# shrubb/latent-pose-reenactment

Measured on AMD Instinct MI355X. Metric: train-step images/sec at 256x256 bs=8, higher is better.
Workload: dtype mixed 16-bit MFMA operands, fp32 accumulate, fp32 activations / weights / optimizer state; 1 GPU; default.yaml meta-training step (configs[2]): ResNeXt50 identity encoder over 8 frames + MobileNetV2 pose encoder (both trained, forward + backward on hand-written gfx950 kernels), G, D with the 98000x512 label embedding, VGG19/VGGFace/featmat/adversarial/dis_embed/dice criterions, Adam, EMA; image_size=256, per_gpu_batch=8, global_batch=8, parallelism=dp1, precision_mode=default assignment (LP_PREC=f16), padding=zero, launch_mode=hipgraph

## Files before the change

include/lp_hip.h:

```cpp
#ifndef LP_HIP_H
#define LP_HIP_H
#include <stdint.h>
#ifdef __cplusplus
extern "C" {
#endif

#define LP_OK 0
#define LP_ERR_ARG (-1)
#define LP_ERR_UNSUPPORTED (-2)
#define LP_ERR_HIP (-3)

#define LP_PREC_BF16 0
#define LP_PREC_BF16X3 1
#define LP_PREC_F16 2

const char* lp_last_error(void);
int lp_abi_version(void);

int lp_pack_weights(const float* w, uint16_t* hi, uint16_t* lo, int Cout, int Cin, int T, int RowsP, int ColsP, int mode, int f16,
                    void* stream);
int lp_pack_desc_bytes(void);
int lp_pack_weights_batch(const void* table, int num_entries, long long total_chunks, void* stream);
int lp_pack_pair_desc_bytes(void);
int lp_pack_weights_pairs(const void* table, int num_entries, long long total_tiles, void* stream);
// ... 184 lines not shown
int lp_reduce_dice(const float* fake, const float* real, float* partial, float* out, float* sums, int B, int Cf, int Cr, int HW,
                   float weight, void* stream);
int lp_reduce_dice_bwd(const float* fake, const float* real, const float* sums, const float* grad_out, float* dfake, int B, int Cf,
                       int Cr, int HW, float weight, void* stream);
int lp_reduce_hinge(const float* real, const float* fake_d, const float* fake_g, float* out, int B, void* stream);
int lp_reduce_hinge_bwd(const float* real, const float* fake_d, const float* grad_G, const float* grad_D, float* d_real,
                        float* d_fake_d, float* d_fake_g, int B, void* stream);

int lp_proj_score_fwd(const float* out, const float* embed, float* pooled, float* dot, int N, int HW, int C, void* stream);
int lp_proj_score_bwd(const float* out, const float* embed, const float* pooled, const float* g_pooled, const float* g_dot, float* d_out,
                      float* d_embed, int N, int HW, int C, void* stream);
int lp_embed_tail_fwd(const float* out, float* elem, float* embeds, int* argk, int B, int K, int HW, int C, int is_max, void* stream);
int lp_embed_tail_bwd(const float* out, const float* g_elem, const float* g_embeds, const int* argk, float* d_out, int B, int K, int HW, int C,
                      int is_max, void* stream);
int lp_stem8_supported(int Cin, int Cout, int ksize, int W);
int lp_stem8_fwd(const float* xa, const long long* stride_a, int Ca, const float* xb, const long long* stride_b, int Cb, int cmap,
                 const uint16_t* w_hi, const uint16_t* w_lo, float* y, const float* bias, const float* alpha, int N, int H, int W, int Cin,
                 int Cout, int CinP, int CoutP, int ksize, int prec, uint16_t* out_hi, uint16_t* out_lo, int out_relu, void* stream);
long long lp_stem8_wgrad_workspace_bytes(int N, int H, int Cout, int ksize);
int lp_stem8_wgrad(const float* xa, const long long* stride_a, int Ca, const float* xb, const long long* stride_b, int Cb, int cmap,
                   const float* dy, float* dw, float* dbias, float* workspace, int N, int H, int W, int Cin, int Cout, int ksize, void* stream);
int lp_stem8_dgrad(const float* dy, const float* w, const float* alpha, float* dx, const long long* stride_dx, int Cb, int cmap, int N, int H,
                   int W, int Cin, int Cout, int ksize, void* stream);
int lp_image_prep_fwd(const float* x, const float* mean, const float* stdv, float* out, int N, int HW, void* stream);
int lp_image_prep_bwd(const float* g, const float* stdv, float* dx, int N, int HW, void* stream);
int lp_stickman_render(const float* points, int N, int P, const int* seg, const int* part_end, const float* colour, int L, int parts, int S,
                       float width, float* out, void* stream);

int lp_mt_desc_bytes(void);
int lp_mt_optimizer_step(const void* table, int num_tensors, long long max_numel, long long* step, int kind, float lr,
                         float beta1, float beta2, float eps, void* stream);
int lp_mt_ema(const void* table, int num_tensors, long long max_numel, float alpha, int copy_only, void* stream);

int lp_sn_desc_bytes(void);
int lp_sn_row_block(void);
int lp_sn_power_iter(const void* table, int num_layers, int do_iter, int max_rows, int max_cols, void* stream);
int lp_sn_grad_apply(float* g, const float* w_orig, const float* u, const float* v, const float* sig, float* dot, int ndot,
                     float* accum, int rows, int cols, void* stream);
int lp_sn_apply_desc_bytes(void);
int lp_sn_grad_apply_batch(const void* host_descs, int count, void* stream);
int lp_sn_embed_grad(float* grad, const float* u, const float* v, const float* coef, const long long* label, const float* rows,
                     int N, int E, int B, void* stream);

#ifdef __cplusplus
}
#endif
// ... 2 lines not shown
```

latent_pose_reenactment_amd/_lib.py:

```python
import ctypes
import os

import torch

_HERE = os.path.dirname(os.path.abspath(__file__))
LIB_PATH = os.environ.get('LP_LIB_OVERRIDE') or os.path.join(_HERE, 'liblp_hip.so')

PREC_BF16 = 0
PREC_BF16X3 = 1
PREC_F16 = 2

_vp, _i, _f, _ll = ctypes.c_void_p, ctypes.c_int, ctypes.c_float, ctypes.c_longlong

SIGNATURES = {
    'lp_last_error': (ctypes.c_char_p, []),
    'lp_abi_version': (_i, []),
    'lp_pack_weights': (_i, [_vp, _vp, _vp, _i, _i, _i, _i, _i, _i, _i, _vp]),
    'lp_pack_desc_bytes': (_i, []),
    'lp_pack_weights_batch': (_i, [_vp, _i, _ll, _vp]),
    'lp_pack_pair_desc_bytes': (_i, []),
    'lp_pack_weights_pairs': (_i, [_vp, _i, _ll, _vp]),
    'lp_act_pack': (_i, [_vp, _vp, _vp, _i, _vp, _vp, _i, _i, _i, _i, _vp, _vp, _i, _i, _vp, _vp]),
    'lp_amax_slots': (_i, []),
    'lp_amax_slot_stride': (_i, []),
# ... 54 lines not shown
    'lp_thin_wgrad16': (_i, [_vp] * 6 + [_i] * 8 + [_vp]),
    'lp_subsample2': (_i, [_vp, _vp, _i, _i, _i, _i, _vp]),
    'lp_zero_stuff2': (_i, [_vp, _vp, _i, _i, _i, _i, _vp]),
    'lp_add_strided2': (_i, [_vp, _vp, _i, _i, _i, _i, _vp]),
    'lp_bn_bwd16_workspace_bytes': (_ll, [_ll, _i]),
    'lp_bn_bwd16': (_i, [_vp] * 14 + [_ll, _i, _i, _f, _i, _i, _vp, _vp]),
    'lp_bn_bwd16_h': (_i, [_vp] * 15 + [_ll, _i, _i, _f, _i, _i, _vp, _vp]),
    'lp_spatial_mean_fwd': (_i, [_vp, _vp, _i, _i, _i, _vp]),
    'lp_spatial_mean_bwd': (_i, [_vp, _vp, _i, _i, _i, _vp]),
    'lp_dwconv3x3_dgrad': (_i, [_vp, _vp, _vp, _i, _i, _i, _i, _i, _vp]),
    'lp_dwconv3x3_wgrad_workspace_bytes': (_ll, [_i]),
    'lp_dwconv3x3_wgrad': (_i, [_vp] * 6 + [_i] * 5 + [_vp]),
    'lp_sum2x2': (_i, [_vp, _vp, _i, _i, _i, _i, _vp, _vp]),
    'lp_sum2x2_planes': (_i, [_vp, _vp, _vp, _vp, _i, _i, _i, _i, _vp]),
    'lp_proj_score_fwd': (_i, [_vp, _vp, _vp, _vp, _i, _i, _i, _vp]),
    'lp_proj_score_bwd': (_i, [_vp, _vp, _vp, _vp, _vp, _vp, _vp, _i, _i, _i, _vp]),
    'lp_embed_tail_fwd': (_i, [_vp] * 4 + [_i] * 5 + [_vp]),
    'lp_embed_tail_bwd': (_i, [_vp] * 5 + [_i] * 5 + [_vp]),
    'lp_stem8_supported': (_i, [_i] * 4),
    'lp_stem8_fwd': (_i, [_vp, _vp, _i, _vp, _vp, _i, _i] + [_vp] * 5 + [_i] * 9 + [_vp, _vp, _i, _vp]),
    'lp_stem8_wgrad_workspace_bytes': (_ll, [_i] * 4),
    'lp_stem8_wgrad': (_i, [_vp, _vp, _i, _vp, _vp, _i, _i] + [_vp] * 4 + [_i] * 6 + [_vp]),
    'lp_stem8_dgrad': (_i, [_vp] * 5 + [_i] * 8 + [_vp]),
    'lp_image_prep_fwd': (_i, [_vp, _vp, _vp, _vp, _i, _i, _vp]),
    'lp_image_prep_bwd': (_i, [_vp, _vp, _vp, _i, _i, _vp]),
    'lp_stickman_render': (_i, [_vp, _i, _i, _vp, _vp, _vp, _i, _i, _i, _f, _vp, _vp]),
    'lp_pool_grad_pack': (_i, [_vp, _vp, _vp, _vp, _vp, _vp, _vp, _i, _i, _i, _i, _i, _vp, _i, _i, _vp, _vp]),
    'lp_adain_relu_bwd_planes': (_i, [_vp, _vp, _vp, _vp, _i, _vp, _vp, _vp, _vp, _vp, _vp, _vp, _vp, _i, _i, _i, _i, _i, _vp, _vp, _i, _vp]),
    'lp_head_fwd': (_i, [_vp, _vp, _vp, _vp, _i, _i, _i, _vp]),
    'lp_head_bwd': (_i, [_vp, _vp, _vp, _vp, _i, _i, _i, _vp, _vp]),
    'lp_tanh_head_fwd': (_i, [_vp, _vp, _vp, _i, _i, _i, _i, _vp]),
    'lp_tanh_head_bwd': (_i, [_vp, _vp, _vp, _i, _i, _i, _i, _vp, _vp]),
    'lp_norm_affine_grad': (_i, [_vp, _vp, _i, _vp, _vp, _i, _i, _i, _vp]),
    'lp_relu_bwd': (_i, [_vp, _vp, _vp, _ll, _vp]),
    'lp_avgpool2_fwd': (_i, [_vp, _vp, _i, _i, _i, _i, _i, _vp, _i, _vp]),
    'lp_avgpool2_fwd16': (_i, [_vp, _vp, _i, _i, _i, _i, _i, _vp]),
    'lp_avgpool2_bwd': (_i, [_vp, _vp, _vp, _i, _i, _i, _i, _i, _vp, _vp]),
    'lp_l1_partial_blocks': (_i, []),
    'lp_l1_fwd': (_i, [_vp, _vp, _vp, _ll, _i, _f, _vp, _vp, _vp]),
    'lp_l1_fwd_b16': (_i, [_vp, _vp, _i, _vp, _ll, _i, _f, _vp, _vp, _vp]),
    'lp_l1_fwd_ab16': (_i, [_vp, _vp, _i, _vp, _ll, _f, _vp, _vp, _vp]),
    'lp_avgpool2_bwd_m16': (_i, [_vp, _vp, _vp, _i, _i, _i, _i, _vp, _vp]),
    'lp_reflect_border_fwd': (_i, [_vp, _vp] + [_i] * 7 + [_vp, _i, _vp, _vp, _vp]),
    'lp_reflect_border_dgrad': (_i, [_vp] + [_i] * 4 + [_vp, _i, _vp, _vp, _i, _vp, _vp]),
    'lp_reflect_border_wgrad': (_i, [_vp, _vp] + [_i] * 7 + [_vp, _i, _vp, _vp, _vp]),
    'lp_reflect_border_wgrad_workspace_bytes': (_ll, [_i] * 5),
# ... 44 lines not shown
```

latent_pose_reenactment_amd/build.py:

```python
import os
import subprocess
import sys
import time
from concurrent.futures import ThreadPoolExecutor

HERE = os.path.dirname(os.path.abspath(__file__))
CSRC = os.path.join(HERE, 'csrc')
INCLUDE = os.path.join(os.path.dirname(HERE), 'include')
LIB = os.path.join(HERE, 'liblp_hip.so')
SOURCES = ['lp_api.hip', 'elementwise.hip', 'norm_bwd.hip', 'tanh_head.hip', 'spectral_norm.hip', 'act_pack.hip', 'conv_dma.hip', 'conv_pipe.hip', 'conv_wgrad.hip', 'conv_thin.hip', 'conv_stem8.hip', 'linear_crop.hip', 'mobilenet.hip', 'resnext.hip', 'reflect_border.hip', 'stickman.hip']
FLAGS = ['--offload-arch=gfx950', '-O3', '-std=c++17', '-fPIC', '-I', INCLUDE, '-I', CSRC]


def _newer(a, b):
    return not os.path.exists(b) or os.path.getmtime(a) > os.path.getmtime(b)


def build(force: bool = False, verbose: bool = True) -> str:
    hipcc = os.environ.get('HIPCC', '/opt/rocm/bin/hipcc')
    objdir = os.path.join(HERE, 'build')
    os.makedirs(objdir, exist_ok=True)
    headers = [os.path.join(CSRC, f) for f in os.listdir(CSRC) if f.endswith('.h')] + [os.path.join(INCLUDE, 'lp_hip.h')]
    jobs = []
    for src in SOURCES:
        s = os.path.join(CSRC, src)
        o = os.path.join(objdir, src.replace('.hip', '.o'))
        if force or _newer(s, o) or any(_newer(h, o) for h in headers):
            jobs.append((s, o))

    def compile_one(job):
        s, o = job
        t_start = time.time()
        cmd = [hipcc] + FLAGS + ['-c', s, '-o', o]
# ... 24 lines not shown
```

latent_pose_reenactment_amd/csrc/conv_wgrad.hip:

```cpp
#include "lp_common.h"
#include "lp_hip.h"
#include "lp_internal.h"
#include <stdlib.h>

struct WgradParams {
    const uint16_t* a_hi; const uint16_t* a_lo; const uint16_t* d_hi; const uint16_t* d_lo; float* part;
    float* bpart;
    int N, H, W, Hin, Win, Cin, Cout, C8, Co8, CoP, CiP;
    int splits, num_tiles;
    int lTH, lTW, lNB, tiles_x, tiles_y;
    int db_acc;
    int diag;
};

__device__ __forceinline__ s16x8_t ld16x8(const uint16_t* p) { return *(const s16x8_t*)p; }
template <bool F16> __device__ __forceinline__ void acc8(float (&s)[8], s16x8_t v) {
#pragma unroll
    for (int j = 0; j < 8; ++j) s[j] += lp_op16_to_f32<F16>((uint16_t)v[j]);
}

typedef s16x4_t __attribute__((address_space(3))) * lds_s16x4_ptr;

__device__ __forceinline__ s16x4_t tr_read(const unsigned char* p) {
    return __builtin_amdgcn_ds_read_tr16_b64_v4i16((lds_s16x4_ptr)(uintptr_t)p);
// ... 527 lines not shown
        for (int nf = 0; nf < 4; ++nf)
#pragma unroll
            for (int r = 0; r < 4; ++r) {
                const int co = co0 + mh * 64 + mf * 16 + (lane >> 4) * 4 + r;
                const int ci = ci0 + nh * 64 + nf * 16 + (lane & 15);
                if (co < p.CoP && ci < p.CiP) slab[(size_t)co * p.CiP + ci] = acc[mf][nf][r];
            }
}

static int launch_wreduce(const WgradParams& p, int T, float* dw, float* dbias, const float* out_scale, const float* sn_w, float* sn_dot,
                          hipStream_t stream) {
    const int bblocks = p.bpart ? (p.Cout + 63) / 64 : 0;
    const int wblocks = wred_blocks(p.Cin, p.Cout, T);
    if (wred_tiled(p.Cin, p.Cout))
        hipLaunchKernelGGL(wgrad_reduce_kernel, dim3(wblocks + bblocks), dim3(256), 0, stream, p.part, dw, p.splits, T, p.Cout, p.Cin, p.CoP, p.CiP,
                           p.bpart, dbias, wblocks, out_scale, sn_w, sn_dot, p.db_acc);
    else if (wred_flat_out(p.Cin, p.Cout, T) == 32)
        hipLaunchKernelGGL(wgrad_reduce_flat_kernel<32>, dim3(wblocks + bblocks), dim3(256), 0, stream, p.part, dw, p.splits, T, p.Cout, p.Cin, p.CoP,
                           p.CiP, p.bpart, dbias, wblocks, out_scale, sn_w, sn_dot, p.db_acc);
    else
        hipLaunchKernelGGL(wgrad_reduce_flat_kernel<256>, dim3(wblocks + bblocks), dim3(256), 0, stream, p.part, dw, p.splits, T, p.Cout, p.Cin, p.CoP,
                           p.CiP, p.bpart, dbias, wblocks, out_scale, sn_w, sn_dot, p.db_acc);
    return lp_check_launch("wgrad_reduce");
}

template <int PREC, int KP>
static int launch_wgrad1x1(WgradParams& p, float* dw, const float* out_scale, const float* sn_w, float* sn_dot, hipStream_t stream) {
    constexpr bool SPLIT = (PREC == LP_PREC_BF16X3);
    W1Params q;
    q.a_hi = p.a_hi; q.a_lo = p.a_lo; q.d_hi = p.d_hi; q.d_lo = p.d_lo; q.part = p.part;
    q.P = (long long)p.N * p.H * p.W;
    q.C8 = p.C8; q.Co8 = p.Co8; q.CoP = p.CoP; q.CiP = p.CiP;
    q.tiles_co = (p.CoP + 127) / 128; q.tiles_ci = (p.CiP + 127) / 128;
    q.nstage = (int)((q.P + KP - 1) / KP);
    int splits = p.splits < q.nstage ? p.splits : q.nstage;
    const int per = (q.nstage + splits - 1) / splits;
    splits = (q.nstage + per - 1) / per;
    p.splits = q.splits = splits;
    q.xcd_map = (splits % 8 == 0);
    const size_t lds = (size_t)2 * KP * 256 * (SPLIT ? 4 : 2);
    auto kern = wgrad1x1_kernel<PREC, KP>;
    static thread_local int attr_dev = -1;
    int dev = 0;
    if (hipGetDevice(&dev) != hipSuccess) return lp_set_error(LP_ERR_HIP, "hipGetDevice failed");
    if (attr_dev != dev) {
        if (hipFuncSetAttribute((const void*)kern, hipFuncAttributeMaxDynamicSharedMemorySize, 160 * 1024) != hipSuccess)
// ... 352 lines not shown
```

latent_pose_reenactment_amd/csrc/lp_internal.h:

```cpp
#pragma once
#include <hip/hip_runtime.h>
#include <stdint.h>
int lp_set_error(int code, const char* msg);
int lp_check_launch(const char* what);

int lp_wgrad_rows_reduce(const float* part, const float* bpart, float* dw, float* dbias, int G, int T, int slabC, int thinC, int wideC, bool thin_x,
                         hipStream_t stream);
```

latent_pose_reenactment_amd/embedders/resnext_hip.py:

```python
import os

import torch

from latent_pose_reenactment_amd import hipops as ops
from latent_pose_reenactment_amd import streams as _streams
from latent_pose_reenactment_amd._lib import PREC_BF16, PREC_BF16X3, PREC_F16


class _BN:
    __slots__ = ('mean', 'rstd', 'scale', 'shift')

    def __init__(self, mean, rstd, scale, shift):
        self.mean, self.rstd, self.scale, self.shift = mean, rstd, scale, shift


def supported(n: int, h: int, w: int) -> bool:
    return h % 32 == 0 and w % 32 == 0 and h >= 128 and w >= 128 and n % 4 == 0 and n >= 8


Y16 = os.environ.get('LP_E_Y16', '1') != '0'
RES16 = os.environ.get('LP_E_RES16', '1') != '0'
MASK16 = os.environ.get('LP_E_MASK16', '1') != '0'


def _side_ok(t):
    return _streams.enabled(t, 'wgrad')


def _v16(a, shape):
    return ops.Act16(a.hi.view(shape), None if a.lo is None else a.lo.view(shape), a.c, a.inv)


def _conv1x1(a16, pack, prec, bias=None, res=None, amax=False, stats=False, y16=False):
    fa = ops.flat16(a16)
    _, h, w, _ = fa.hi.shape
    if res is not None:
        res = res.view(1, h, w, -1)
    if y16:
        out = ops.conv16(fa, pack, ksize=1, bias=bias, res=res, prec=prec, stats=stats, want_y=False, out16=0, kind='conv1x1')
        return out[1:] if stats else out[1]
    return ops.conv16(fa, pack, ksize=1, bias=bias, res=res, prec=prec, amax=amax, stats=stats, kind='conv1x1')


def _yview(y, shape):
    return _v16(y, shape) if isinstance(y, ops.Act16) else y.view(shape)
# ... 23 lines not shown
class ResNeXtFunction(torch.autograd.Function):

    @staticmethod
    def forward(ctx, net, x, *params):
        prec = net.prec
        train = net.training
        need_grad = any(ctx.needs_input_grad[2:])
        if ctx.needs_input_grad[1]:
            raise RuntimeError('the HIP encoder does not differentiate with respect to its input frames (detach them)')
        par = dict(zip(net._hip_param_names, params))
        packs = net._hip_packs(par, need_grad)
        bn_eval = None if train else net._hip_eval_affines(par)
        counters = []

        def bn(y, name, st=None):
            if not train:
                return bn_eval[name]
            return bn_state(y, st, par[name + '.weight'].detach(), par[name + '.bias'].detach(), net._hip_bn[name], counters)

        n, _, hin, win = x.shape
        x = x.detach().contiguous()
        if x.dtype not in (torch.float32, torch.float64):
            x = x.float()
        cols = ops.im2col_planes(x, 7, 2, 3, prec)
        h0, w0 = cols.hi.shape[1], cols.hi.shape[2]
        y0, cs = _conv1x1(cols, packs['conv1.weight'][0], prec, stats=True)
        y0 = y0.view(n, h0, w0, 64)
        st0 = bn(y0, 'bn1', cs)
        bprecs = net.block_precs()
        lprecs = net.layer_precs()
        out, out16, idx = ops.bn_relu_maxpool(y0, st0.scale, st0.shift, lprecs[(net._hip_blocks[0][0], 'conv1')], want_idx=need_grad)
        saved_blocks = []
        base_prec = prec
        nblk = len(net._hip_blocks)

        def next_prec(b):
            return lprecs[(net._hip_blocks[b + 1][0], 'conv1')] if b + 1 < nblk else bprecs[b]
        planes_res = [RES16 and MASK16 and not blk[5] and lprecs[(blk[0], 'conv1')] in (PREC_BF16, PREC_BF16X3) and next_prec(b) == lprecs[(blk[0], 'conv1')]
                      for b, blk in enumerate(net._hip_blocks)]
        for bi, (bname, cin, width, cout, stride, down) in enumerate(net._hip_blocks):
            prec = bprecs[bi]
            p1, p2, p3 = lprecs[(bname, 'conv1')], lprecs[(bname, 'conv2')], lprecs[(bname, 'conv3')]
            nprec = lprecs[(net._hip_blocks[bi + 1][0], 'conv1')] if bi + 1 < len(bprecs) else prec
            y16 = Y16 and p1 == p2 == p3 == PREC_F16
            assert not (y16 and nprec != PREC_F16), 'an fp16 block must be followed by fp16 blocks (lp_bn_add_act16 writes fp16 planes)'
            xin, xin16 = out, out16
            _, h, w, _ = xin16.hi.shape
            y1, cs = _conv1x1(xin16, packs[bname + '.conv1.weight'][0], p1, stats=True, y16=y16)
            y1 = _yview(y1, (n, h, w, width))
            st1 = bn(y1, bname + '.bn1', cs)
# ... 18 lines not shown
                yd, cs = _conv1x1(xd16, packs[bname + '.downsample.0.weight'][0], p1, stats=True)
                yd = yd.view(n, ho, wo, cout)
                std = bn(yd, bname + '.downsample.1', cs)
                need_f32 = bi + 1 >= nblk or not (net._hip_blocks[bi + 1][5] or planes_res[bi + 1])
                out, out16 = ops.bn_add_act(y3, st3.scale, st3.shift, yd, std.scale, std.shift, relu=True, prec=nprec, want_out=need_f32 or not MASK16)
            elif planes_res[bi]:
                need_f32 = bi + 1 >= nblk or not (net._hip_blocks[bi + 1][5] or planes_res[bi + 1])
                out, out16 = ops.bn_add_act(y3, st3.scale, st3.shift, xin16, relu=True, prec=nprec, want_out=need_f32)
            else:
                out, out16 = ops.bn_add_act(y3, st3.scale, st3.shift, xin, relu=True, prec=nprec)
            if need_grad:
                saved_blocks.append((xin16, y1, st1, a1, y2, st2, a2, y3, st3, xd16, yd, std, out16 if MASK16 else (out16 if y16 else out), (h, w, ho, wo), (p1, p2, p3)))
        prec = base_prec
        _, hl, wl, cl = out.shape
        pooled = ops.spatial_mean(out)
        fh, fw = ops.flat_hw(n)
        p16 = ops.act_pack(pooled.view(1, fh, fw, cl), pro=0, prec=prec)
        logits = ops.conv16(p16, packs['fc.weight'][0], ksize=1, bias=par['fc.bias'].detach().contiguous(), prec=prec).view(n, -1)
        if counters:
            torch._foreach_add_(counters, 1)
        if need_grad:
            ctx.params = params
            ctx.net, ctx.par, ctx.packs, ctx.train = net, par, packs, train
            ctx.stem = (cols, y0, st0, idx, (h0, w0))
            ctx.blocks = saved_blocks
            ctx.head = (p16, (hl, wl, cl), (fh, fw))
            ctx.n = n
        return logits

    @staticmethod
    def backward(ctx, d_logits):
        if ctx.blocks is None:
            raise RuntimeError('backward through the HIP encoder a second time: its saved activations were released by the first pass (retain_graph is not supported)')
        net, par, packs, train = ctx.net, ctx.par, ctx.packs, ctx.train
        prec = net.prec
        frozen = not train
        n = ctx.n
        grads = {}

        def bn_bwd(dA, y, st, name, prec=None, **kw):
            prec = net.prec if prec is None else prec
            d16, dg, db, g = ops.bn_bwd16(dA, y, par[name + '.weight'].detach(), st.mean, st.rstd, st.scale, st.shift, prec=prec, frozen=frozen, **kw)
            grads[name + '.weight'], grads[name + '.bias'] = dg, db
            return d16, g

        wside = _side_ok(d_logits)
        keep = []
# ... 18 lines not shown
            wgrad(bname + '.conv3.weight', lambda a, d, k=bname + '.conv3.weight', p=p3: _wgrad1x1(a, d, p).view(par[k].shape), a2, d16)
            dA2 = _conv1x1(d16, packs[bname + '.conv3.weight'][1], p3).view(n, ho, wo, width)
            d16, _ = bn_bwd(dA2, y2, st2, bname + '.bn2', p2)
            if stride == 2:
                d16 = ops.zero_stuff2_16(d16, h, w)
            cg = par[bname + '.conv2.weight'].shape[1]
            wgrad(bname + '.conv2.weight', lambda a, d, cg=cg, p=p2: ops.gconv_wgrad16(a, d, cg, prec=p), a1, d16)
            dA1 = ops.gconv16(d16, packs[bname + '.conv2.weight'][1], prec=p2)
            d16, _ = bn_bwd(dA1, y1, st1, bname + '.bn1', p1)
            wgrad(bname + '.conv1.weight', lambda a, d, k=bname + '.conv1.weight', p=p1: _wgrad1x1(a, d, p).view(par[k].shape), xin16, d16)
            if down:
                dd16, _ = bn_bwd(d_out, yd, std, bname + '.downsample.1', p1, mask_mode=2, mask_src=out)
                wgrad(bname + '.downsample.0.weight', lambda a, d, k=bname + '.downsample.0.weight', p=p1: _wgrad1x1(a, d, p).view(par[k].shape), xd16, dd16)
                d_xd = _conv1x1(dd16, packs[bname + '.downsample.0.weight'][1], p1)
                if stride == 2:
                    d_xin = _conv1x1(d16, packs[bname + '.conv1.weight'][1], p1).view(n, h, w, cin)
                    ops.add_strided2(d_xin, d_xd.view(n, ho, wo, cin))
                else:
                    d_xin = _conv1x1(d16, packs[bname + '.conv1.weight'][1], p1, res=d_xd).view(n, h, w, cin)
            else:
                d_xin = _conv1x1(d16, packs[bname + '.conv1.weight'][1], p1, res=g).view(n, h, w, cin)
            d_out = d_xin
        prec = net.prec
        cols, y0, st0, idx, (h0, w0) = ctx.stem
        dA0 = ops.maxpool_bwd(d_out, idx, h0, w0)
        d16, _ = bn_bwd(dA0, y0, st0, 'bn1')
        wgrad('conv1.weight', lambda a, d: _wgrad1x1(a, d, prec).view(par['conv1.weight'].shape), cols, d16)
        if wside:
            torch.cuda.current_stream(d_logits.device).wait_stream(_streams.side_stream(d_logits.device, 4))
        keep.clear()
        ctx.blocks = ctx.stem = ctx.head = None
        from latent_pose_reenactment_amd.nn import fused_accumulate
        return (None, None) + tuple(fused_accumulate(ctx.params, [grads.get(k) for k in net._hip_param_names]))
```

latent_pose_reenactment_amd/hipops.py:

```python
import os
from typing import NamedTuple, Optional, Tuple

import torch

from . import _lib
from ._lib import PREC_BF16, PREC_BF16X3, PREC_F16, check
from .dataloaders.synthetic_voxceleb2_stickmen import PARTS

Tensor = torch.Tensor


def _stream():
    return torch.cuda.current_stream().cuda_stream


PROFILE = None


class _Timed:
    def __init__(self, kind, flops, tag=None, nbytes=0.0, mm=1):
        self.mm = mm
        self.rw = tuple(nbytes) if isinstance(nbytes, tuple) else None
        self.kind, self.flops, self.tag, self.nbytes = kind, flops, tag, (sum(nbytes) if isinstance(nbytes, tuple) else nbytes)

# ... 360 lines not shown
    ws = torch.empty(_lib.lib().lp_stem8_wgrad_workspace_bytes(n, h, cout, ksize) // 4, dtype=torch.float32, device=dy.device)
    dw = torch.empty((cout, cin, ksize, ksize), dtype=torch.float32, device=dy.device)
    db = torch.empty(cout, dtype=torch.float32, device=dy.device) if bias_grad else None
    (a, keep_a), (b, keep_b) = _src4(xa, 'xa'), _src4(xb, 'xb')
    with _Timed('wgrad_thin', 2.0 * n * h * w * cout * cin * ksize * ksize, (n, h, w, cin, cout, ksize, 0, 0), (n * h * w * (cout + cin) * 4, dw.numel() * 4)):
        check(_lib.lib().lp_stem8_wgrad(*a, *b, _c_int32(cmap), dy.data_ptr(), dw.data_ptr(), _p(db), ws.data_ptr(), n, h, w, cin, cout, ksize,
                                        _stream()), 'lp_stem8_wgrad')
    dw = _sn_finish(dw, sn, accum)
    return (dw, db) if bias_grad else dw


def stem8_dgrad(dy: Tensor, w_orig: Tensor, alpha: Optional[Tensor], cmap: int, cb: int, *, ksize: int) -> Tensor:
    _chk(dy, 'dy'); _chk(w_orig, 'w_orig')
    n, h, w, cout = dy.shape
    cin = w_orig.shape[1]
    dx = torch.empty((n, cb, h, w), dtype=torch.float32, device=dy.device)
    (_, dx_strides, _), keep = _src4(dx, 'dx')
    with _Timed('conv_thin', 2.0 * n * h * w * cout * cb * ksize * ksize, (n, h, w, cout, cb, ksize, 0, 0), (dy.numel() * 4, dx.numel() * 4)):
        check(_lib.lib().lp_stem8_dgrad(dy.data_ptr(), w_orig.data_ptr(), _p(alpha), dx.data_ptr(), dx_strides, cb, _c_int32(cmap), n, h, w,
                                        cin, cout, ksize, _stream()), 'lp_stem8_dgrad')
    return dx


def embed_tail_fwd(out: Tensor, b: int, k: int, use_max: bool):
    _chk(out, 'out')
    bk, h, w, c = out.shape
    assert bk == b * k, (out.shape, b, k)
    elem = torch.empty((b, k, c), dtype=torch.float32, device=out.device)
    embeds = torch.empty((b, c), dtype=torch.float32, device=out.device)
    argk = torch.empty((b, c), dtype=torch.int32, device=out.device) if use_max else None
    check(_lib.lib().lp_embed_tail_fwd(out.data_ptr(), elem.data_ptr(), embeds.data_ptr(), _p(argk), b, k, h * w, c, int(use_max), _stream()), 'lp_embed_tail_fwd')
    return elem, embeds, argk


def embed_tail_bwd(out: Tensor, g_elem: Optional[Tensor], g_embeds: Optional[Tensor], argk: Optional[Tensor], b: int, k: int, use_max: bool) -> Tensor:
    for t, nm in ((g_elem, 'g_elem'), (g_embeds, 'g_embeds')):
        if t is not None:
            _chk(t, nm)
    bk, h, w, c = out.shape
    d_out = torch.empty_like(out)
    check(_lib.lib().lp_embed_tail_bwd(out.data_ptr(), _p(g_elem), _p(g_embeds), _p(argk), d_out.data_ptr(), b, k, h * w, c, int(use_max), _stream()),
          'lp_embed_tail_bwd')
    return d_out


def conv(x: Tensor, pack: WeightPack, *, ksize: int, upsample: bool = False, pro: int = 0, scale: Optional[Tensor] = None,
# ... 1084 lines not shown
```

Baseline: 198.1 images/s.

## Add direct implicit-im2col 7x7 stem conv kernels for ResNeXt encoder

Replaces the ResNeXt stem path, which ran an explicit im2col_planes followed by a 1x1 GEMM, with a dedicated 7x7 stride-2 kernel. The new kernel stages each input patch into LDS directly from the NCHW fp32 image and computes per-tile BN statistics in the epilogue. A matching weight-gradient kernel reads the raw image plus the 16-bit dy planes and writes per-block slabs that are reduced afterwards. This avoids materialising and re-reading the large column buffer in both forward and backward, at the cost of new hand-tuned kernels whose LDS gathers may be less efficient than the generic GEMM.

```diff
diff --git a/include/lp_hip.h b/include/lp_hip.h
--- a/include/lp_hip.h
+++ b/include/lp_hip.h
@@ -230,6 +230,12 @@
                    const float* dy, float* dw, float* dbias, float* workspace, int N, int H, int W, int Cin, int Cout, int ksize, void* stream);
 int lp_stem8_dgrad(const float* dy, const float* w, const float* alpha, float* dx, const long long* stride_dx, int Cb, int cmap, int N, int H,
                    int W, int Cin, int Cout, int ksize, void* stream);
+long long lp_stem7_stats_rows(int N, int H, int W);
+int lp_stem7_fwd(const float* x, const uint16_t* w_hi, const uint16_t* w_lo, float* y, float* stats, int N, int C, int H, int W, int Cout, int CinP,
+                 int CoutP, int ksize, int stride, int pad, int prec, void* stream);
+long long lp_stem7_wgrad_workspace_bytes(int N, int H, int W);
+int lp_stem7_wgrad(const float* x, const uint16_t* d_hi, const uint16_t* d_lo, float* dw, float* workspace, const float* out_scale, int N, int C,
+                   int H, int W, int Cout, int ksize, int stride, int pad, int prec, void* stream);
 int lp_image_prep_fwd(const float* x, const float* mean, const float* stdv, float* out, int N, int HW, void* stream);
 int lp_image_prep_bwd(const float* g, const float* stdv, float* dx, int N, int HW, void* stream);
 int lp_stickman_render(const float* points, int N, int P, const int* seg, const int* part_end, const float* colour, int L, int parts, int S,
diff --git a/latent_pose_reenactment_amd/_lib.py b/latent_pose_reenactment_amd/_lib.py
--- a/latent_pose_reenactment_amd/_lib.py
+++ b/latent_pose_reenactment_amd/_lib.py
@@ -100,6 +100,10 @@
     'lp_stem8_wgrad_workspace_bytes': (_ll, [_i] * 4),
     'lp_stem8_wgrad': (_i, [_vp, _vp, _i, _vp, _vp, _i, _i] + [_vp] * 4 + [_i] * 6 + [_vp]),
     'lp_stem8_dgrad': (_i, [_vp] * 5 + [_i] * 8 + [_vp]),
+    'lp_stem7_stats_rows': (_ll, [_i] * 3),
+    'lp_stem7_fwd': (_i, [_vp] * 5 + [_i] * 11 + [_vp]),
+    'lp_stem7_wgrad_workspace_bytes': (_ll, [_i] * 3),
+    'lp_stem7_wgrad': (_i, [_vp] * 6 + [_i] * 9 + [_vp]),
     'lp_image_prep_fwd': (_i, [_vp, _vp, _vp, _vp, _i, _i, _vp]),
     'lp_image_prep_bwd': (_i, [_vp, _vp, _vp, _i, _i, _vp]),
     'lp_stickman_render': (_i, [_vp, _i, _i, _vp, _vp, _vp, _i, _i, _i, _f, _vp, _vp]),
diff --git a/latent_pose_reenactment_amd/build.py b/latent_pose_reenactment_amd/build.py
--- a/latent_pose_reenactment_amd/build.py
+++ b/latent_pose_reenactment_amd/build.py
@@ -8,7 +8,7 @@
 CSRC = os.path.join(HERE, 'csrc')
 INCLUDE = os.path.join(os.path.dirname(HERE), 'include')
 LIB = os.path.join(HERE, 'liblp_hip.so')
-SOURCES = ['lp_api.hip', 'elementwise.hip', 'norm_bwd.hip', 'tanh_head.hip', 'spectral_norm.hip', 'act_pack.hip', 'conv_dma.hip', 'conv_pipe.hip', 'conv_wgrad.hip', 'conv_thin.hip', 'conv_stem8.hip', 'linear_crop.hip', 'mobilenet.hip', 'resnext.hip', 'reflect_border.hip', 'stickman.hip']
+SOURCES = ['lp_api.hip', 'elementwise.hip', 'norm_bwd.hip', 'tanh_head.hip', 'spectral_norm.hip', 'act_pack.hip', 'conv_dma.hip', 'conv_pipe.hip', 'conv_wgrad.hip', 'conv_thin.hip', 'conv_stem8.hip', 'conv_stem7.hip', 'linear_crop.hip', 'mobilenet.hip', 'resnext.hip', 'reflect_border.hip', 'stickman.hip']
 FLAGS = ['--offload-arch=gfx950', '-O3', '-std=c++17', '-fPIC', '-I', INCLUDE, '-I', CSRC]
 
 
diff --git a/latent_pose_reenactment_amd/csrc/conv_stem7.hip b/latent_pose_reenactment_amd/csrc/conv_stem7.hip
--- /dev/null
+++ b/latent_pose_reenactment_amd/csrc/conv_stem7.hip
@@ -0,0 +1,421 @@
+#include "lp_common.h"
+#include "lp_hip.h"
+#include "lp_internal.h"
+
+#if defined(__HIP_DEVICE_COMPILE__)
+#pragma clang attribute push(__attribute__((target("no-packed-fp32-ops"))), apply_to = function)
+#endif
+
+__device__ __forceinline__ void stem7_barrier() { asm volatile("s_waitcnt lgkmcnt(0)\n\ts_barrier" ::: "memory"); }
+__device__ __forceinline__ float stem7_shfl_xor(float v, int o) {
+    return __builtin_bit_cast(float, __builtin_amdgcn_ds_bpermute((int)(((threadIdx.x & 63) ^ o) << 2), __builtin_bit_cast(int, v)));
+}
+
+constexpr int S7_K = 147, S7_KP = 160, S7_CO = 64, S7_TP = 64;
+constexpr int S7_PROWS = 21, S7_PHALF = 68, S7_PROW = 136;
+constexpr int S7_PCOLS = 133;
+constexpr int S7_PWORDS = S7_PROWS * S7_PROW;
+constexpr int S7_ZERO = S7_PWORDS;
+constexpr int S7_DUMMY = S7_ZERO + 72;
+constexpr int S7_PATCH_B = (S7_PWORDS + 72 + 4) * 4;
+constexpr int S7_NLD = (S7_PWORDS + 255) / 256;
+constexpr int S7_WROW = 168;
+constexpr int S7_DROW = 144;
+constexpr int S7_MAXWG = 512;
+
+struct Stem7Params {
+    const float* x; const uint16_t* w_hi; const uint16_t* w_lo; float* y; float* stats;
+    const uint16_t* d_hi; const uint16_t* d_lo; float* part;
+    int N, H, W, Ho, Wo, tpr, ntiles, CinP, per;
+};
+
+struct Stem7Tile { int n, oy, ox0, npx; };
+
+__device__ __forceinline__ Stem7Tile stem7_tile(const Stem7Params& p, int t) {
+    Stem7Tile q;
+    const int tx = t % p.tpr, r = t / p.tpr;
+    q.oy = r % p.Ho; q.n = r / p.Ho; q.ox0 = tx * S7_TP; q.npx = min(S7_TP, p.Wo - q.ox0);
+    return q;
+}
+
+__device__ __forceinline__ int stem7_tap_word(int k) {
+    if (k >= S7_K) return S7_ZERO;
+    const int row = k / 7, kx = k - row * 7;
+    return row * S7_PROW + (kx & 1) * S7_PHALF + (kx >> 1);
+}
+
+struct Stem7Stage { int goff[S7_NLD], meta[S7_NLD]; };
+template <int NT> struct Stem7Nld { static constexpr int N = (S7_PWORDS + NT - 1) / NT; };
+
+template <int NT>
+__device__ __forceinline__ void stem7_stage_init(const Stem7Params& p, int tid, Stem7Stage& s) {
+#pragma unroll
+    for (int i = 0; i < Stem7Nld<NT>::N; ++i) {
+        const int e = tid + i * NT;
+        const int r = e / S7_PROW, j = e - r * S7_PROW;
+        const int c = r / 7, ky = r - c * 7;
+        const bool el = e < S7_PWORDS && j < S7_PCOLS;
+        const int lw = e < S7_PWORDS ? r * S7_PROW + (j & 1) * S7_PHALF + (j >> 1) : S7_DUMMY;
+        s.goff[i] = el ? (c * p.H + ky) * p.W + j : 0;
+        s.meta[i] = j | (el ? ky : 7) << 8 | lw << 12;
+    }
+}
+
+template <int NT>
+__device__ __forceinline__ unsigned stem7_patch_load(const Stem7Params& p, const Stem7Tile& t, const Stem7Stage& s, float (&v)[S7_NLD]) {
+    unsigned rowmask = 0, okmask = 0;
+#pragma unroll
+    for (int ky = 0; ky < 7; ++ky) { const int iy = 2 * t.oy - 3 + ky; rowmask |= (iy >= 0 && iy < p.H) ? 1u << ky : 0u; }
+    const int jlo = 3 - 2 * t.ox0, jhi = p.W + 3 - 2 * t.ox0;
+    const long long base = ((long long)t.n * 3 * p.H + 2 * t.oy - 3) * p.W + 2 * t.ox0 - 3;
+#pragma unroll
+    for (int i = 0; i < Stem7Nld<NT>::N; ++i) {
+        const int j = s.meta[i] & 255, ky = (s.meta[i] >> 8) & 7;
+        const bool ok = ((rowmask >> ky) & 1u) && j >= jlo && j < jhi;
+        v[i] = p.x[ok ? base + s.goff[i] : 0];
+        okmask |= ok ? 1u << i : 0u;
+    }
+    return okmask;
+}
+
+template <bool F16, bool SPLIT, int NT>
+__device__ __forceinline__ void stem7_patch_store(unsigned* patch, const Stem7Stage& s, const float (&v)[S7_NLD], unsigned okmask) {
+#pragma unroll
+    for (int i = 0; i < Stem7Nld<NT>::N; ++i) {
+        const float q = (okmask >> i) & 1u ? v[i] : 0.f;
+        const uint16_t h = lp_f32_to_op16<F16>(q);
+        unsigned w = h;
+        if (SPLIT) w |= (unsigned)lp_f32_to_op16<false>(q - lp_op16_to_f32<false>(h)) << 16;
+        patch[(unsigned)s.meta[i] >> 12] = w;
+    }
+}
+
+__device__ __forceinline__ void stem7_split8(const unsigned (&w)[8], s16x8_t& hi, s16x8_t& lo) {
+#pragma unroll
+    for (int j = 0; j < 8; ++j) { hi[j] = (short)(w[j] & 0xffffu); lo[j] = (short)(w[j] >> 16); }
+}
+
+template <int MODE>
+__global__ __launch_bounds__(256, 2) void conv_stem7_fwd_kernel(Stem7Params p) {
+    constexpr bool F16 = MODE == LP_PREC_F16, X3 = MODE == LP_PREC_BF16X3;
+    constexpr int W_PLANE_B = S7_CO * S7_WROW * 2;
+    extern __shared__ __attribute__((aligned(16))) unsigned char smem[];
+    unsigned* patch = (unsigned*)smem;
+    const uint16_t* Wh = (const uint16_t*)(smem + S7_PATCH_B);
+    const uint16_t* Wl = (const uint16_t*)(smem + S7_PATCH_B + W_PLANE_B);
+    const int tid = threadIdx.x, lane = tid & 63, wave = tid >> 6;
+    float* Tall = (float*)(smem + S7_PATCH_B + W_PLANE_B * (X3 ? 2 : 1));
+    float* Tl = Tall + wave * (16 * 68);
+    const int kg = lane >> 4, m = lane & 15;
+
+    for (int e = tid; e < S7_CO * 20; e += 256) {
+        const int co = e / 20, ch = e - co * 20;
+        *(s16x8_t*)(smem + S7_PATCH_B + (co * S7_WROW + ch * 8) * 2) = *(const s16x8_t*)(p.w_hi + (size_t)co * p.CinP + ch * 8);
+        if (X3) *(s16x8_t*)(smem + S7_PATCH_B + W_PLANE_B + (co * S7_WROW + ch * 8) * 2) = *(const s16x8_t*)(p.w_lo + (size_t)co * p.CinP + ch * 8);
+    }
+    for (int e = tid; e < 72; e += 256) patch[S7_ZERO + e] = 0u;
+
+    int aw[5][8];
+#pragma unroll
+    for (int ks = 0; ks < 5; ++ks)
+#pragma unroll
+        for (int j = 0; j < 8; ++j) {
+            const int k = ks * 32 + kg * 8 + j;
+            aw[ks][j] = stem7_tap_word(k) + (k < S7_K ? wave * 16 + m : 0);
+        }
+    const int boff = m * S7_WROW + kg * 8;
+
+    auto tile_stats = [&](int st_t, int st_npx) {
+        const int ch = tid >> 2, rs = tid & 3;
+        float st_n = 0.f, st_ref = 0.f, st_d = 0.f, st_q = 0.f;
+#pragma unroll
+        for (int i = 0; i < 16; ++i) {
+            const int row = rs + 4 * i;
+            if (row < st_npx) {
+                const float v = Tall[row * 68 + ch];
+                if (st_n == 0.f) st_ref = v;
+                const float d = v - st_ref;
+                st_d += d; st_q = fmaf(d, d, st_q);
+                st_n += 1.f;
+            }
+        }
+        float mean = 0.f, m2 = 0.f;
+        if (st_n > 0.f) { mean = st_ref + st_d / st_n; m2 = fmaxf(st_q - st_d * st_d / st_n, 0.f); }
+#pragma unroll
+        for (int o = 1; o < 4; o <<= 1) {
+            const float nb_ = stem7_shfl_xor(st_n, o);
+            const float mb = stem7_shfl_xor(mean, o), qb = stem7_shfl_xor(m2, o);
+            const float nn = st_n + nb_;
+            if (nn > 0.f) {
+                const float fb = nb_ / nn, fab = st_n * fb;
+                const float d = mb - mean; mean = fmaf(d, fb, mean); m2 += qb + d * d * fab;
+            }
+            st_n = nn;
+        }
+        if (rs == 0) { float* o = p.stats + ((size_t)st_t * S7_CO + ch) * 3; o[0] = st_n; o[1] = mean; o[2] = m2; }
+    };
+    int st_t = -1, st_npx = 0;
+    Stem7Stage stg;
+    stem7_stage_init<256>(p, tid, stg);
+    float pv[S7_NLD];
+    int t = blockIdx.x;
+    Stem7Tile cur = stem7_tile(p, t);
+    unsigned pok = stem7_patch_load<256>(p, cur, stg, pv);
+    for (; t < p.ntiles; t += gridDim.x) {
+        stem7_barrier();
+        if (p.stats && st_t >= 0) tile_stats(st_t, st_npx);
+        stem7_patch_store<F16, X3, 256>(patch, stg, pv, pok);
+        stem7_barrier();
+        const Stem7Tile tl = cur;
+        if (t + (int)gridDim.x < p.ntiles) { cur = stem7_tile(p, t + gridDim.x); pok = stem7_patch_load<256>(p, cur, stg, pv); }
+        const bool live = wave * 16 < tl.npx;
+        f32x4_t acc[4];
+#pragma unroll
+        for (int nt = 0; nt < 4; ++nt) acc[nt] = (f32x4_t){0.f, 0.f, 0.f, 0.f};
+        if (live) {
+#pragma unroll
+        for (int ks = 0; ks < 5; ++ks) {
+            unsigned w[8];
+#pragma unroll
+            for (int j = 0; j < 8; ++j) w[j] = patch[aw[ks][j]];
+            s16x8_t ah, al;
+            stem7_split8(w, ah, al);
+#pragma unroll
+            for (int nt = 0; nt < 4; ++nt) {
+                const int o = boff + nt * 16 * S7_WROW + ks * 32;
+                const s16x8_t bh = *(const s16x8_t*)(Wh + o);
+                if (X3) {
+                    const s16x8_t bl = *(const s16x8_t*)(Wl + o);
+                    acc[nt] = mfma16(al, bh, acc[nt]);
+                    acc[nt] = mfma16(ah, bl, acc[nt]);
+                }
+                acc[nt] = mfma16t<F16>(ah, bh, acc[nt]);
+            }
+        }
+        }
+#pragma unroll
+        for (int nt = 0; nt < 4; ++nt)
+#pragma unroll
+            for (int q = 0; q < 4; ++q) Tl[(kg * 4 + q) * 68 + nt * 16 + m] = acc[nt][q];
+        __builtin_amdgcn_fence(__ATOMIC_ACQ_REL, "wavefront");
+        const size_t pix0 = ((size_t)tl.n * p.Ho + tl.oy) * p.Wo + tl.ox0 + wave * 16;
+#pragma unroll
+        for (int i = 0; i < 4; ++i) {
+            const int row = i * 4 + kg;
+            const float4 v = *(const float4*)(Tl + row * 68 + m * 4);
+            if (wave * 16 + row < tl.npx) *(float4*)(p.y + (pix0 + row) * S7_CO + m * 4) = v;
+        }
+        st_t = t; st_npx = tl.npx;
+    }
+    if (p.stats && st_t >= 0) { stem7_barrier(); tile_stats(st_t, st_npx); }
+}
+
+typedef s16x4_t __attribute__((address_space(3))) * s7_lds_s16x4_ptr;
+__device__ __forceinline__ s16x4_t stem7_tr_read(const unsigned char* q) {
+    return __builtin_amdgcn_ds_read_tr16_b64_v4i16((s7_lds_s16x4_ptr)(uintptr_t)q);
+}
+
+__device__ __forceinline__ void stem7_dy_load(const Stem7Params& p, const Stem7Tile& t, const uint16_t* plane, int tid, s16x8_t (&v)[1]) {
+    const size_t pix0 = ((size_t)t.n * p.Ho + t.oy) * p.Wo + t.ox0;
+#pragma unroll
+    for (int i = 0; i < 1; ++i) {
+        const int e = tid, px = e >> 3, c8 = e & 7;
+        v[i] = *(const s16x8_t*)(plane + (pix0 + min(px, t.npx - 1)) * S7_CO + c8 * 8);
+    }
+}
+__device__ __forceinline__ void stem7_dy_store(unsigned char* D, int tid, const s16x8_t (&v)[1], int npx) {
+#pragma unroll
+    for (int i = 0; i < 1; ++i) {
+        const int e = tid, px = e >> 3, c8 = e & 7;
+        const s16x8_t z = {0, 0, 0, 0, 0, 0, 0, 0};
+        *(s16x8_t*)(D + px * S7_DROW + c8 * 16) = px < npx ? v[i] : z;
+    }
+}
+
+template <int MODE>
+__global__ __launch_bounds__(512, 2) void wgrad_stem7_kernel(Stem7Params p) {
+    constexpr bool F16 = MODE == LP_PREC_F16, X3 = MODE == LP_PREC_BF16X3;
+    constexpr int D_PLANE_B = S7_TP * S7_DROW;
+    extern __shared__ __attribute__((aligned(16))) unsigned char smem[];
+    unsigned* patch = (unsigned*)smem;
+    unsigned char* Dh = smem + S7_PATCH_B;
+    unsigned char* Dl = Dh + D_PLANE_B;
+    const int tid = threadIdx.x, lane = tid & 63, wave8 = __builtin_amdgcn_readfirstlane(tid >> 6);
+    const int wave = wave8 & 3, mh = wave8 >> 2;
+    const int G = lane >> 4, n16 = lane & 15;
+    for (int e = tid; e < 72; e += 512) patch[S7_ZERO + e] = 0u;
+
+    int bw[3];
+#pragma unroll
+    for (int i = 0; i < 3; ++i) bw[i] = stem7_tap_word(min(wave + 4 * i, 9) * 16 + n16) + G * 4;
+    const bool third = wave < 2;
+    const int sj = n16 >> 2, sq = lane & 3;
+    const int doff = (G * 4 + sj) * S7_DROW + sq * 8 + mh * 64;
+
+    f32x4_t acc[2][3];
+#pragma unroll
+    for (int mf = 0; mf < 2; ++mf)
+#pragma unroll
+        for (int i = 0; i < 3; ++i) acc[mf][i] = (f32x4_t){0.f, 0.f, 0.f, 0.f};
+
+    Stem7Stage stg;
+    stem7_stage_init<512>(p, tid, stg);
+    float pv[S7_NLD];
+    s16x8_t dh[1], dl[1];
+    int t = blockIdx.x * p.per;
+    const int t_end = min(p.ntiles, t + p.per);
+    Stem7Tile cur = stem7_tile(p, t);
+    unsigned pok = stem7_patch_load<512>(p, cur, stg, pv);
+    stem7_dy_load(p, cur, p.d_hi, tid, dh);
+    if (X3) stem7_dy_load(p, cur, p.d_lo, tid, dl);
+    for (; t < t_end; ++t) {
+        stem7_barrier(); 
+        stem7_patch_store<F16, X3, 512>(patch, stg, pv, pok);
+        stem7_dy_store(Dh, tid, dh, cur.npx);
+        if (X3) stem7_dy_store(Dl, tid, dl, cur.npx);
+        stem7_barrier(); 
+        if (t + 1 < t_end) {
+            cur = stem7_tile(p, t + 1);
+            pok = stem7_patch_load<512>(p, cur, stg, pv);
+            stem7_dy_load(p, cur, p.d_hi, tid, dh);
+            if (X3) stem7_dy_load(p, cur, p.d_lo, tid, dl);
+        }
+#pragma unroll
+        for (int ks = 0; ks < 2; ++ks) {
+            s16x8_t fa[2], fal[2];
+#pragma unroll
+            for (int mf = 0; mf < 2; ++mf) {
+                const unsigned char* a0 = Dh + ks * 32 * S7_DROW + doff + mf * 32;
+                const s16x4_t v0 = stem7_tr_read(a0), v1 = stem7_tr_read(a0 + 16 * S7_DROW);
+                fa[mf] = (s16x8_t){v0[0], v0[1], v0[2], v0[3], v1[0], v1[1], v1[2], v1[3]};
+                if (X3) {
+                    const s16x4_t x0 = stem7_tr_read(a0 + D_PLANE_B), x1 = stem7_tr_read(a0 + D_PLANE_B + 16 * S7_DROW);
+                    fal[mf] = (s16x8_t){x0[0], x0[1], x0[2], x0[3], x1[0], x1[1], x1[2], x1[3]};
+                }
+            }
+#pragma unroll
+            for (int i = 0; i < 3; ++i) {
+                if (i == 2 && !third) continue;
+                unsigned w[8];
+#pragma unroll
+                for (int j = 0; j < 4; ++j) { w[j] = patch[bw[i] + ks * 32 + j]; w[4 + j] = patch[bw[i] + ks * 32 + 16 + j]; }
+                s16x8_t fb, fbl;
+                stem7_split8(w, fb, fbl);
+#pragma unroll
+                for (int mf = 0; mf < 2; ++mf) {
+                    if (X3) {
+                        acc[mf][i] = mfma16(fal[mf], fb, acc[mf][i]);
+                        acc[mf][i] = mfma16(fa[mf], fbl, acc[mf][i]);
+                    }
+                    acc[mf][i] = mfma16t<F16>(fa[mf], fb, acc[mf][i]);
+                }
+            }
+        }
+    }
+    float* slab = p.part + (size_t)blockIdx.x * S7_CO * S7_KP;
+#pragma unroll
+    for (int i = 0; i < 3; ++i) {
+        if (i == 2 && !third) continue;
+#pragma unroll
+        for (int mf = 0; mf < 2; ++mf)
+#pragma unroll
+            for (int r = 0; r < 4; ++r) slab[((mh * 2 + mf) * 16 + G * 4 + r) * S7_KP + (wave + 4 * i) * 16 + n16] = acc[mf][i][r];
+    }
+}
+
+static bool stem7_geometry(int C, int Cout, int ksize, int stride, int pad, int H, int W) {
+    return C == 3 && Cout == S7_CO && ksize == 7 && stride == 2 && pad == 3 && H >= 7 && W >= 7;
+}
+
+static bool stem7_fill(Stem7Params& p, int N, int H, int W) {
+    p.N = N; p.H = H; p.W = W; p.Ho = (H - 1) / 2 + 1; p.Wo = (W - 1) / 2 + 1;
+    p.tpr = (p.Wo + S7_TP - 1) / S7_TP;
+    const long long nt = (long long)N * p.Ho * p.tpr;
+    if (nt > 0x7fffffffll - S7_MAXWG || (long long)N * p.Ho * p.Wo * S7_CO > 0x7fffffff00ll || 3ll * H * W > 0x7fffffffll) return false;
+    p.ntiles = (int)nt;
+    return true;
+}
+
+static int stem7_groups(int ntiles) { return ntiles < S7_MAXWG ? ntiles : S7_MAXWG; }
+
+static void stem7_wgrad_ranges(int ntiles, int& G, int& per) {
+    int s = ntiles / 8;
+    if (s > 256) s = 256;
+    if (s < 1) s = 1;
+    if (s >= 8) s = s / 8 * 8;
+    per = (ntiles + s - 1) / s;
+    G = (ntiles + per - 1) / per;
+}
+
+template <typename K> static int stem7_lds_attr(K kern, size_t lds) {
+    if (lds <= 64 * 1024) return LP_OK;
+    if (hipFuncSetAttribute((const void*)kern, hipFuncAttributeMaxDynamicSharedMemorySize, (int)lds) != hipSuccess)
+        return lp_set_error(LP_ERR_HIP, "hipFuncSetAttribute failed");
+    return LP_OK;
+}
+
+extern "C" long long lp_stem7_stats_rows(int N, int H, int W) {
+    Stem7Params p;
+    if (N < 1 || H < 7 || W < 7 || !stem7_fill(p, N, H, W)) return 0;
+    return p.ntiles;
+}
+
+extern "C" int lp_stem7_fwd(const float* x, const uint16_t* w_hi, const uint16_t* w_lo, float* y, float* stats, int N, int C, int H, int W, int Cout,
+                            int CinP, int CoutP, int ksize, int stride, int pad, int prec, void* stream) {
+    if (!x || !w_hi || !y) return lp_set_error(LP_ERR_ARG, "lp_stem7_fwd: null pointer");
+    if (prec != LP_PREC_BF16 && prec != LP_PREC_BF16X3 && prec != LP_PREC_F16) return lp_set_error(LP_ERR_ARG, "lp_stem7_fwd: unknown operand mode");
+    if (prec == LP_PREC_BF16X3 && !w_lo) return lp_set_error(LP_ERR_ARG, "lp_stem7_fwd: bf16x3 needs the lo plane");
+    if (N < 1) return lp_set_error(LP_ERR_ARG, "lp_stem7_fwd: empty tensor");
+    if (!stem7_geometry(C, Cout, ksize, stride, pad, H, W)) return lp_set_error(LP_ERR_UNSUPPORTED, "lp_stem7_fwd: needs 3 -> 64 channels, 7x7, stride 2, pad 3, H, W >= 7");
+    if (CinP < S7_KP || (CinP % 8) != 0 || CoutP < S7_CO) return lp_set_error(LP_ERR_ARG, "lp_stem7_fwd: weight pack geometry");
+    Stem7Params p = {};
+    if (!stem7_fill(p, N, H, W)) return lp_set_error(LP_ERR_UNSUPPORTED, "lp_stem7_fwd: tensor too large");
+    p.x = x; p.w_hi = w_hi; p.w_lo = w_lo; p.y = y; p.stats = stats; p.CinP = CinP;
+    using Kernel = void (*)(Stem7Params);
+    static const Kernel kernels[3] = {conv_stem7_fwd_kernel<LP_PREC_BF16>, conv_stem7_fwd_kernel<LP_PREC_BF16X3>, conv_stem7_fwd_kernel<LP_PREC_F16>};
+    static_assert(LP_PREC_BF16 == 0 && LP_PREC_BF16X3 == 1 && LP_PREC_F16 == 2, "the kernel table is indexed by the operand mode");
+    const size_t lds = S7_PATCH_B + (size_t)S7_CO * S7_WROW * 2 * (prec == LP_PREC_BF16X3 ? 2 : 1) + (size_t)4 * 16 * 68 * sizeof(float);
+    static thread_local int attr_dev[3] = {-1, -1, -1};
+    int dev = 0;
+    if (hipGetDevice(&dev) != hipSuccess) return lp_set_error(LP_ERR_HIP, "hipGetDevice failed");
+    if (attr_dev[prec] != dev) {
+        const int rc = stem7_lds_attr(kernels[prec], lds);
+        if (rc) return rc;
+        attr_dev[prec] = dev;
+    }
+    hipLaunchKernelGGL(kernels[prec], dim3(stem7_groups(p.ntiles)), dim3(256), lds, (hipStream_t)stream, p);
+    return lp_check_launch("conv_stem7_fwd");
+}
+
+extern "C" long long lp_stem7_wgrad_workspace_bytes(int N, int H, int W) {
+    Stem7Params p;
+    if (N < 1 || H < 7 || W < 7 || !stem7_fill(p, N, H, W)) return 0;
+    int G, per;
+    stem7_wgrad_ranges(p.ntiles, G, per);
+    return (long long)G * S7_CO * S7_KP * (long long)sizeof(float);
+}
+
+extern "C" int lp_stem7_wgrad(const float* x, const uint16_t* d_hi, const uint16_t* d_lo, float* dw, float* workspace, const float* out_scale, int N,
+                              int C, int H, int W, int Cout, int ksize, int stride, int pad, int prec, void* stream) {
+    if (!x || !d_hi || !dw || !workspace) return lp_set_error(LP_ERR_ARG, "lp_stem7_wgrad: null pointer");
+    if (prec != LP_PREC_BF16 && prec != LP_PREC_BF16X3 && prec != LP_PREC_F16) return lp_set_error(LP_ERR_ARG, "lp_stem7_wgrad: unknown operand mode");
+    if (prec == LP_PREC_BF16X3 && !d_lo) return lp_set_error(LP_ERR_ARG, "lp_stem7_wgrad: bf16x3 needs the lo plane");
+    if (N < 1) return lp_set_error(LP_ERR_ARG, "lp_stem7_wgrad: empty tensor");
+    if (!stem7_geometry(C, Cout, ksize, stride, pad, H, W)) return lp_set_error(LP_ERR_UNSUPPORTED, "lp_stem7_wgrad: needs 3 -> 64 channels, 7x7, stride 2, pad 3, H, W >= 7");
+    Stem7Params p = {};
+    if (!stem7_fill(p, N, H, W)) return lp_set_error(LP_ERR_UNSUPPORTED, "lp_stem7_wgrad: tensor too large");
+    p.x = x; p.d_hi = d_hi; p.d_lo = d_lo; p.part = workspace;
+    using Kernel = void (*)(Stem7Params);
+    static const Kernel kernels[3] = {wgrad_stem7_kernel<LP_PREC_BF16>, wgrad_stem7_kernel<LP_PREC_BF16X3>, wgrad_stem7_kernel<LP_PREC_F16>};
+    int G;
+    stem7_wgrad_ranges(p.ntiles, G, p.per);
+    const size_t lds = S7_PATCH_B + (size_t)S7_TP * S7_DROW * (prec == LP_PREC_BF16X3 ? 2 : 1);
+    hipLaunchKernelGGL(kernels[prec], dim3(G), dim3(512), lds, (hipStream_t)stream, p);
+    const int rc = lp_check_launch("wgrad_stem7");
+    if (rc) return rc;
+    return lp_wgrad_reduce_slabs(workspace, G, S7_K, S7_CO, S7_CO, S7_KP, dw, out_scale, (hipStream_t)stream);
+}
+
+#if defined(__HIP_DEVICE_COMPILE__)
+#pragma clang attribute pop
+#endif
diff --git a/latent_pose_reenactment_amd/csrc/conv_wgrad.hip b/latent_pose_reenactment_amd/csrc/conv_wgrad.hip
--- a/latent_pose_reenactment_amd/csrc/conv_wgrad.hip
+++ b/latent_pose_reenactment_amd/csrc/conv_wgrad.hip
@@ -573,6 +573,12 @@
         hipLaunchKernelGGL(wgrad_reduce_flat_kernel<256>, dim3(wblocks + bblocks), dim3(256), 0, stream, p.part, dw, p.splits, T, p.Cout, p.Cin, p.CoP,
                            p.CiP, p.bpart, dbias, wblocks, out_scale, sn_w, sn_dot, p.db_acc);
     return lp_check_launch("wgrad_reduce");
+}
+
+int lp_wgrad_reduce_slabs(const float* part, int splits, int Cin, int Cout, int CoP, int CiP, float* dw, const float* out_scale, hipStream_t stream) {
+    WgradParams p = {};
+    p.part = const_cast<float*>(part); p.splits = splits; p.Cin = Cin; p.Cout = Cout; p.CoP = CoP; p.CiP = CiP;
+    return launch_wreduce(p, 1, dw, nullptr, out_scale, nullptr, nullptr, stream);
 }
 
 template <int PREC, int KP>
diff --git a/latent_pose_reenactment_amd/csrc/lp_internal.h b/latent_pose_reenactment_amd/csrc/lp_internal.h
--- a/latent_pose_reenactment_amd/csrc/lp_internal.h
+++ b/latent_pose_reenactment_amd/csrc/lp_internal.h
@@ -6,3 +6,5 @@
 
 int lp_wgrad_rows_reduce(const float* part, const float* bpart, float* dw, float* dbias, int G, int T, int slabC, int thinC, int wideC, bool thin_x,
                          hipStream_t stream);
+
+int lp_wgrad_reduce_slabs(const float* part, int splits, int Cin, int Cout, int CoP, int CiP, float* dw, const float* out_scale, hipStream_t stream);
diff --git a/latent_pose_reenactment_amd/embedders/resnext_hip.py b/latent_pose_reenactment_amd/embedders/resnext_hip.py
--- a/latent_pose_reenactment_amd/embedders/resnext_hip.py
+++ b/latent_pose_reenactment_amd/embedders/resnext_hip.py
@@ -20,7 +20,12 @@
 
 Y16 = os.environ.get('LP_E_Y16', '1') != '0'
 RES16 = os.environ.get('LP_E_RES16', '1') != '0'
+STEM_DIRECT = os.environ.get('LP_E_STEM_DIRECT', '1') != '0'
 MASK16 = os.environ.get('LP_E_MASK16', '1') != '0'
+
+
+def _stem_direct():
+    return STEM_DIRECT and hasattr(ops, 'stem7_conv') and hasattr(ops, 'stem7_wgrad')
 
 
 def _side_ok(t):
@@ -90,10 +95,15 @@
         x = x.detach().contiguous()
         if x.dtype not in (torch.float32, torch.float64):
             x = x.float()
-        cols = ops.im2col_planes(x, 7, 2, 3, prec)
-        h0, w0 = cols.hi.shape[1], cols.hi.shape[2]
-        y0, cs = _conv1x1(cols, packs['conv1.weight'][0], prec, stats=True)
-        y0 = y0.view(n, h0, w0, 64)
+        if _stem_direct():
+            stem_in = x
+            y0, cs = ops.stem7_conv(x, packs['conv1.weight'][0], prec=prec, stats=True)
+            h0, w0 = y0.shape[1], y0.shape[2]
+        else:
+            stem_in = ops.im2col_planes(x, 7, 2, 3, prec)
+            h0, w0 = stem_in.hi.shape[1], stem_in.hi.shape[2]
+            y0, cs = _conv1x1(stem_in, packs['conv1.weight'][0], prec, stats=True)
+            y0 = y0.view(n, h0, w0, 64)
         st0 = bn(y0, 'bn1', cs)
         bprecs = net.block_precs()
         lprecs = net.layer_precs()
@@ -158,7 +168,7 @@
         if need_grad:
             ctx.params = params
             ctx.net, ctx.par, ctx.packs, ctx.train = net, par, packs, train
-            ctx.stem = (cols, y0, st0, idx, (h0, w0))
+            ctx.stem = (stem_in, y0, st0, idx, (h0, w0))
             ctx.blocks = saved_blocks
             ctx.head = (p16, (hl, wl, cl), (fh, fw))
             ctx.n = n
@@ -223,10 +233,13 @@
                 d_xin = _conv1x1(d16, packs[bname + '.conv1.weight'][1], p1, res=g).view(n, h, w, cin)
             d_out = d_xin
         prec = net.prec
-        cols, y0, st0, idx, (h0, w0) = ctx.stem
+        stem_in, y0, st0, idx, (h0, w0) = ctx.stem
         dA0 = ops.maxpool_bwd(d_out, idx, h0, w0)
         d16, _ = bn_bwd(dA0, y0, st0, 'bn1')
-        wgrad('conv1.weight', lambda a, d: _wgrad1x1(a, d, prec).view(par['conv1.weight'].shape), cols, d16)
+        if isinstance(stem_in, ops.Act16):
+            wgrad('conv1.weight', lambda a, d: _wgrad1x1(a, d, prec).view(par['conv1.weight'].shape), stem_in, d16)
+        else:
+            wgrad('conv1.weight', lambda a, d: ops.stem7_wgrad(a, d, prec=prec), stem_in, d16)
         if wside:
             torch.cuda.current_stream(d_logits.device).wait_stream(_streams.side_stream(d_logits.device, 4))
         keep.clear()
diff --git a/latent_pose_reenactment_amd/hipops.py b/latent_pose_reenactment_amd/hipops.py
--- a/latent_pose_reenactment_amd/hipops.py
+++ b/latent_pose_reenactment_amd/hipops.py
@@ -406,6 +406,41 @@
     return dx
 
 
+def stem7_conv(x: Tensor, pack: WeightPack, *, prec: int, stats: bool = False):
+    _chk(x, 'x')
+    n, c, h, w = x.shape
+    ho, wo = (h - 1) // 2 + 1, (w - 1) // 2 + 1
+    cout = pack.rows
+    assert pack.cols == c * 49 and pack.taps == 1, (pack.rows, pack.cols, pack.taps)
+    y = torch.empty((n, ho, wo, cout), dtype=torch.float32, device=x.device)
+    st, rows = None, 0
+    if stats:
+        rows = _lib.lib().lp_stem7_stats_rows(n, h, w)
+        st = torch.empty((max(rows, 1), cout, 3), dtype=torch.float32, device=x.device)
+    pl = 4 if prec == PREC_BF16X3 else 2
+    with _Timed('conv_stem7', 2.0 * n * ho * wo * cout * c * 49, (n, ho, wo, c, cout, 7, 0, 0), (x.numel() * 4 + pack.hi.numel() * pl, y.numel() * 4),
+                mm=3 if prec == PREC_BF16X3 else 1):
+        check(_lib.lib().lp_stem7_fwd(x.data_ptr(), pack.hi.data_ptr(), _p(pack.lo), y.data_ptr(), _p(st), n, c, h, w, cout, pack.cols_p, pack.rows_p,
+                                      7, 2, 3, prec, _stream()), 'lp_stem7_fwd')
+    return (y, ConvStats(st, rows, 1)) if stats else y
+
+
+def stem7_wgrad(x: Tensor, dy: Act16, *, prec: int) -> Tensor:
+    _chk(x, 'x')
+    n, c, h, w = x.shape
+    ho, wo = (h - 1) // 2 + 1, (w - 1) // 2 + 1
+    cout = dy.c
+    assert dy.nhw == (n, ho, wo) and dy.hi.shape[3] == cout and dy.hi.is_contiguous(), (dy.hi.shape, x.shape)
+    ws = torch.empty(max(_lib.lib().lp_stem7_wgrad_workspace_bytes(n, h, w) // 4, 1), dtype=torch.float32, device=x.device)
+    dw = torch.empty((cout, c, 7, 7), dtype=torch.float32, device=x.device)
+    pl = 4 if prec == PREC_BF16X3 else 2
+    with _Timed('wgrad_stem7', 2.0 * n * ho * wo * cout * c * 49, (n, ho, wo, c, cout, 7, 0, 0), (x.numel() * 4 + dy.hi.numel() * pl, dw.numel() * 4),
+                mm=3 if prec == PREC_BF16X3 else 1):
+        check(_lib.lib().lp_stem7_wgrad(x.data_ptr(), dy.hi.data_ptr(), _p(dy.lo), dw.data_ptr(), ws.data_ptr(), _p(dy.inv), n, c, h, w, cout,
+                                        7, 2, 3, prec, _stream()), 'lp_stem7_wgrad')
+    return dw
+
+
 def embed_tail_fwd(out: Tensor, b: int, k: int, use_max: bool):
     _chk(out, 'out')
     bk, h, w, c = out.shape
```

Result: no change. 200.3 images/s (median of 6 runs) (+1.1%).
